# KalistaW/enterprise_warp

Hardware: AMD Instinct MI355X
Metric: lnL evals/sec (whole node), 45-psr CURN batched; % fp64 MFMA peak (higher is better)
Workload: dtype f64; 1 GPU; C3: 45 psr, n=2000..20000 TOAs (495k) over 14.7 yr, ECORR, RN+DM 30 freqs, CURN 14 freqs merged, fixed white noise (TNT cached), basis m=132; global_batch=4096, batch_per_gpu=4096, n_pulsars=45, parallelism=units1

## Files before the change

### enterprise_warp_amd/_lib.py

```python
import ctypes as C
import os

_HERE = os.path.dirname(os.path.abspath(__file__))
CPU_LIB_PATH = os.path.join(_HERE, "libewarp_cpu.so")
BACKEND = os.environ.get("EWARP_BACKEND", "hip").lower()
if BACKEND not in ("hip", "cpu"):
    raise ValueError(f"EWARP_BACKEND={BACKEND!r}: expected 'hip' (default) or 'cpu'")
LIB_PATH = os.environ.get("EWARP_HIP_LIB") or (CPU_LIB_PATH if BACKEND == "cpu" else
                                               os.path.join(_HERE, "libewarp_hip.so"))
DEV_LIB_PATH = os.path.join(_HERE, "libewarp_hip_dev.so")

EWH_ABI_VERSION = 11
COMMON_MAX_TERMS = 16
COMMON_CORRELATED, COMMON_OPTSTAT = 0, 1
SPEC_POWERLAW, SPEC_TURNOVER, SPEC_FREESPEC, SPEC_CONST = 1, 2, 3, 4
DELAY_EXP_DIP, DELAY_YEARLY_SIN = 1, 2


class Pref(C.Structure):
    _fields_ = [("idx", C.c_int32), ("pad_", C.c_int32), ("cval", C.c_double)]


class SpecEntry(C.Structure):
    _fields_ = [("kind", C.c_int32), ("col", C.c_int32), ("p0", Pref), ("p1", Pref), ("p2", Pref),
# ... 29 lines not shown
    _fields_ = [("n_col", C.c_int32), ("orf", _dp), ("spec", C.POINTER(SpecEntry)), ("kind", C.c_int32),
                ("n_term", C.c_int32), ("terms", C.POINTER(CommonTerm))]


class PtaDesc(C.Structure):
    _fields_ = [("abi_version", C.c_int32), ("n_pulsar", C.c_int32), ("n_param", C.c_int32),
                ("white_fixed", C.c_int32), ("pulsars", C.POINTER(PulsarDesc)), ("common", C.POINTER(CommonDesc))]


EXPORTS = ["ewh_create", "ewh_num_devices", "ewh_set_fixed_white", "ewh_lnl_batch", "ewh_lnl_units_device",
           "ewh_keep_dim", "ewh_corr_partial_device", "ewh_corr_finish_device",
           "ewh_last_unit_terms", "ewh_unit_cost", "ewh_set_kernel_mode", "ewh_optstat", "ewh_contract_device",
           "ewh_transfer_stats", "ewh_lat_b_max", "ewh_refine_stats", "ewh_cond_dims", "ewh_cond_gp",
           "ewh_cond_joint_dims", "ewh_cond_joint",
           "ewh_destroy", "ewh_last_error", "ewh_version"]
DEV_EXPORTS = ["ewh_dev_gram", "ewh_dev_reduced", "ewh_dev_images"]

_lib = None


class EngineError(RuntimeError):
    pass


def load():
    global _lib
    if _lib is not None:
        return _lib
    if BACKEND != "cpu":
        try:
            import torch
# ... 52 lines not shown
    lib.ewh_lat_b_max.argtypes = []
    lib.ewh_lat_b_max.restype = C.c_int
    lib.ewh_destroy.argtypes = [C.c_void_p]
    lib.ewh_destroy.restype = None
    lib.ewh_last_error.argtypes = []
    lib.ewh_last_error.restype = C.c_char_p
    lib.ewh_version.argtypes = []
    lib.ewh_version.restype = C.c_int
    if hasattr(lib, "ewh_dev_gram"):
        lib.ewh_dev_gram.argtypes = [C.c_void_p, C.c_int32, _dp, C.c_int32, _dp]
        lib.ewh_dev_gram.restype = C.c_int
        lib.ewh_dev_reduced.argtypes = [C.c_void_p, C.c_int32, _dp, _dp]
        lib.ewh_dev_reduced.restype = C.c_int
        lib.ewh_dev_images.argtypes = [C.c_void_p, C.c_int32, _dp, _dp, _ip]
        lib.ewh_dev_images.restype = C.c_int
    _lib = lib
    return lib


def check(rc):
    if rc != 0:
        raise EngineError(f"libewarp_hip error {rc}: {_lib.ewh_last_error().decode(errors='replace')}")
```

### enterprise_warp_amd/csrc/chol_partial.hip

```cpp
#include "ewarp_dev.h"

namespace ewh_dev {
namespace {

template <int NB, int KEEP>
int launch_partial(const UnitSpan& s, double* keep_out, int keep_bs) {
  if constexpr (partial_in_registers(NB, KEEP) && NB - KEEP >= Split<NB>::H) {
    hipLaunchKernelGGL(HIP_KERNEL_NAME(chol_mfma_kernel<NB, default_waves(NB), PANEL_2L, false, KEEP>),
                       dim3((unsigned)s.n), dim3(64), 0, s.st, s.jobs, s.B, s.u0, s.b_off, s.theta, s.ldth, s.units,
                       keep_out, 0, keep_bs);
    return 0;
  } else {
    return set_err(EWH_E_UNSUPPORTED, "common: reduced basis too narrow for the kept common block");
  }
}

}

int launch_partial_nb(int nb, int keep, const UnitSpan& s, double* keep_out, int keep_bs) {
  if (!partial_in_registers(nb, keep))
    return set_err(EWH_E_UNSUPPORTED, "common: no register kernel for this reduced width and kept size");
#define EWH_PARTK(NBV, KV) \
  case KV: return launch_partial<NBV, KV>(s, keep_out, keep_bs);
#define EWH_PART(NBV)   \
  case NBV:             \
// ... 26 lines not shown
```

### enterprise_warp_amd/csrc/chol_small.hip

```cpp
#include "ewarp_dev.h"

namespace ewh_dev {
namespace {

static_assert(front_map_ok(1) && front_map_ok(2) && front_map_ok(3) && front_map_ok(4) && front_map_ok(5) &&
                  front_map_ok(6) && front_map_ok(7) && front_map_ok(8) && front_map_ok(9),
              "front-pad map: a permutation of the frame, real columns and r in order, pads onto stored pads");
static_assert(MFMA_NB_MAX == 9, "front_map_ok covers every register-kernel width");
static_assert(front_elem_ok(1) && front_elem_ok(2) && front_elem_ok(3) && front_elem_ok(4) && front_elem_ok(5) &&
                  front_elem_ok(6) && front_elem_ok(7) && front_elem_ok(8) && front_elem_ok(9),
              "front_elem: base + constant + lane part == front_src(row) LD + front_src(col)");
static_assert(img_map_ok(1) && img_map_ok(2) && img_map_ok(3), "operand image map, 1..3 blocks");
static_assert(img_map_ok(4) && img_map_ok(5), "operand image map, 4 and 5 blocks");
static_assert(img_map_ok(6), "operand image map, 6 blocks");
static_assert(img_map_ok(7), "operand image map, 7 blocks");
static_assert(img_map_ok(8), "operand image map, 8 blocks");
static_assert(img_map_ok(9), "operand image map, 9 blocks");

template <int NB, int ALG = PANEL_2L, bool STAMP = false, int W = default_waves(NB), bool FULL = false, int DEAD = -1,
          bool IMG = false>
void launch_chol_mfma(const UnitSpan& s) {
  hipLaunchKernelGGL(HIP_KERNEL_NAME(chol_mfma_kernel<NB, W, ALG, STAMP, 0, FULL, DEAD, IMG>), dim3((unsigned)s.n),
                     dim3(64), 0, s.st, s.jobs, s.B, s.u0, s.b_off, s.theta, s.ldth, s.units, nullptr, 0, 0);
}

template <int NB, bool STAMP = false, bool IMG = false>
void launch_chol_front(int dead, const UnitSpan& s) {
  constexpr int W = default_waves(NB);
  switch (front_inst(NB, dead)) {
    case 3: launch_chol_mfma<NB, PANEL_2L, STAMP, W, false, 3, IMG>(s); break;
    case 2: launch_chol_mfma<NB, PANEL_2L, STAMP, W, false, 2, IMG>(s); break;
    case 1: launch_chol_mfma<NB, PANEL_2L, STAMP, W, false, NB == 6 ? -1 : 1, IMG>(s); break;
    default: launch_chol_mfma<NB, PANEL_2L, STAMP, W, false, -1, IMG>(s); break;
  }
}

template <int NB, bool STAMP = false>
void launch_chol_product(int dead, bool img, const UnitSpan& s) {
  if (img)
    launch_chol_front<NB, STAMP, true>(dead, s);
  else
    launch_chol_front<NB, STAMP, false>(dead, s);
}

}

#ifdef EWH_DEV
bool variant_built(int mode) {
  return mode == 15 || mode == 16 || mode == 17 || mode == 19 || mode == 21 || mode == 22 || mode == 23 ||
         mode == 24 || mode == 25 || mode == 26 || mode == 28 || mode == 30 || mode == 31 || mode == 32;
}
extern "C" int ewh_dev_stamps(long long* out, long long n) {
  if (n > (long long)STAMP_UNITS * STAMP_N) n = (long long)STAMP_UNITS * STAMP_N;
  return hipMemcpyFromSymbol(out, HIP_SYMBOL(g_stamps), (size_t)n * sizeof(long long)) == hipSuccess ? 0 : -1;
}
#else
bool variant_built(int) { return false; }
#endif

int launch_chol_small(int mode, int nb, int dead, bool img, const UnitSpan& s) {
#ifdef EWH_DEV
  if (nb == 8) {
    switch (mode) {
      case 17: launch_chol_mfma<8, PANEL_1L>(s); return 0;
      case 21: launch_chol_product<8, true>(dead, img, s); return 0;
      case 26: launch_chol_mfma<8, PANEL_2L, false, 1, true>(s); return 0;
      default: break;
    }
  }
#endif
  switch (nb) {
    case 1: launch_chol_product<1>(dead, img, s); return 0;
    case 2: launch_chol_product<2>(dead, img, s); return 0;
    case 3: launch_chol_product<3>(dead, img, s); return 0;
    case 4: launch_chol_product<4>(dead, img, s); return 0;
    case 5: launch_chol_product<5>(dead, img, s); return 0;
    case 6: launch_chol_product<6>(dead, img, s); return 0;
    case 7: launch_chol_product<7>(dead, img, s); return 0;
    case 8: launch_chol_product<8>(dead, img, s); return 0;
    case 9: launch_chol_product<9>(dead, img, s); return 0;
    default: return set_err(EWH_E_UNSUPPORTED, "no register kernel past 9 blocks");
  }
}

}
```

### enterprise_warp_amd/csrc/ewarp_ctx.h

```cpp
#pragma once

#include "ewarp_launch.h"
#include "ewarp_mem.h"

#include <utility>

namespace ewh_host {

using namespace ewh_dev;
using namespace ewh_mem;

constexpr size_t LDS_MAX = 160 * 1024;

struct PsrHost {
  int n_toa = 0, m = 0, nlead = 0, ld = 0, nb = 0, n_epoch = 0;
  int max_epoch = 0;
  int fx_m = 0, fx_ld = 0, fx_nb = 0;
  int ncommon = 0, nloc = 0, gstart = 0;
  int gstart_v = 0;
  PsrDev dev{};
  int* d_colptr = nullptr;
  DSpec* d_spec = nullptr;
  int* d_fx_colptr = nullptr;
  DSpec* d_fx_spec = nullptr;
  int* d_fx_rep = nullptr;
  int* d_fx_ulist = nullptr;
  int fx_nu = 0;
  URec* d_fx_urec = nullptr;
  std::vector<int> fx_tidx;
  int* d_fx_urep = nullptr;
  double* d_S = nullptr;
  double* d_Slo = nullptr;
  double* d_Srev = nullptr;
  double* d_img = nullptr;
  double* d_imgf = nullptr;
  double* d_Tlo = nullptr;
  bool has_theta_white = false;
  int n_slot = 0;
  ewh_pref* d_slots = nullptr;
  std::vector<ewh_pref> slots;
  DelayDev delay{};
  double *d_Gf = nullptr, *d_Gflo = nullptr, *d_wf = nullptr, *d_betaf = nullptr;
  double fxKb = 0.0;
  int nproj = 0;
  bool has_proj = false;
// ... 163 lines not shown
```

### enterprise_warp_amd/csrc/ewarp_dev.h

```cpp
#pragma once
#include <hip/hip_runtime.h>

#include <algorithm>
#include <cmath>
#include <cstdint>
#include <cstring>
#include <string>
#include <type_traits>
#include <vector>

#include "ewarp_hip.h"
#include "ewarp_route.h"

namespace ewh_dev {

int set_err(int code, const std::string& msg);

#define EWH_HIP(expr)                                                          \
  do {                                                                         \
    hipError_t e_ = (expr);                                                    \
    if (e_ != hipSuccess)                                                      \
      return ::ewh_dev::set_err(EWH_E_HIP, std::string(#expr) + ": " + hipGetErrorString(e_)); \
  } while (0)

#ifdef EWH_DEBUG
#define EWH_DCHECK(cond, what)                                                                           \
  do {                                                                                                   \
// ... 27 lines not shown
}

struct DSpec {
  int kind, col;
  int i0, i1, i2, pad_;
  double v0, v1, v2;
  double a, lnf, lnfyr, f;
};

__device__ __forceinline__ double dpar(int idx, double cval, const double* th) {
  return idx >= 0 ? th[idx] : cval;
}

constexpr double LN10 = 2.302585092994045684;

template <int DUMMY = 0>
__device__ __forceinline__ double spec_phi_body(const DSpec& s, const double* th) {
  switch (s.kind) {
    case EWH_SPEC_POWERLAW: {
      const double lgA = dpar(s.i0, s.v0, th), gam = dpar(s.i1, s.v1, th);
      return exp(s.a + 2.0 * LN10 * lgA + (gam - 3.0) * s.lnfyr - gam * s.lnf);
    }
    case EWH_SPEC_TURNOVER: {
      const double lgA = dpar(s.i0, s.v0, th), gam = dpar(s.i1, s.v1, th);
      double fc = dpar(s.i2, s.v2, th);
      if (fc < 0) fc = exp(LN10 * fc);
      return exp(s.a + 2.0 * LN10 * lgA - 3.0 * s.lnfyr - gam * (log(s.f + fc) - s.lnfyr));
    }
    case EWH_SPEC_FREESPEC:
      return exp(2.0 * LN10 * dpar(s.i0, s.v0, th));
    case EWH_SPEC_CONST:
      return s.v0;
    default:
      return __builtin_nan("");
  }
}
// ... 148 lines not shown
  const DSpec* spec;
  const double* K;
  int kstride;
  int fail;
  const int* rep = nullptr;
  const int* ulist = nullptr;
  int nu = 0;
  const struct URec* urec = nullptr;
  const int* urep = nullptr;
  int ntidx = 0;
  int tidx[16] = {};
  const double* mats_lo = nullptr;
  const double* mats_rev = nullptr;
  const double* img = nullptr;
  const double* img_front = nullptr;
};

struct UnitSpan {
  const CholJob* jobs; int B; long long u0, n; int b_off;
  const double* theta; int ldth; double* units; hipStream_t st;
};

struct URec {
  static constexpr int NE = 3;
  DSpec e[NE];
  int ne, pad_[3];
};
constexpr int STAGE_THETA_MAX = 512;
constexpr int TIDX_MAX = 16;

template <int NB>
__global__ __launch_bounds__(256) void contract_mfma_kernel(PsrDev P, const double* __restrict__ w,
                                                            const double* __restrict__ beta,
                                                            const double* __restrict__ s,
                                                            const double* __restrict__ fac,
                                                            double* __restrict__ G) {
  constexpr int LD = 16 * NB;
  constexpr int NBLK = NB * (NB + 1) / 2;
  constexpr int SLOTS = (NBLK + 3) / 4;
  extern __shared__ __attribute__((aligned(16))) double smem[];
  double* tile = smem;
  double* wt = smem + CT_ROWS * LD;
// ... 388 lines not shown
#pragma unroll
  for (int sk = S0; sk < 4; ++sk) C = __builtin_amdgcn_mfma_f64_16x16x4f64(Ui[sk], Uj[sk], C, 0, 0, 1);
}

constexpr int FRONT_PAD_MAX = 15;
__host__ __device__ constexpr int front_pads(int ld, int mreal) {
  const int s = ld - 1 - mreal;
  return s < 0 ? 0 : s > FRONT_PAD_MAX ? FRONT_PAD_MAX : s;
}
__host__ __device__ constexpr int front_src(int w, int s, int ld) {
  return w < s ? ld - 1 - s + w : w == ld - 1 ? w : w - s;
}
constexpr int front_dead(int ld, int mreal) { return front_pads(ld, mreal) / 4; }
constexpr int front_inst(int nb, int dead) {
  return dead <= 0 || (nb == 6 && dead == 1) ? -1 : dead > 3 ? 3 : dead;
}
constexpr bool front_map_ok(int nb) {
  const int ld = 16 * nb;
  for (int mreal = 0; mreal < ld; ++mreal) {
    const int s = front_pads(ld, mreal);
    int next = 0;
    for (int w = 0; w < ld; ++w) {
      const int a = front_src(w, s, ld);
      if (w < s) {
        if (a != ld - 1 - s + w || a < mreal || a >= ld - 1) return false;
      } else if (w == ld - 1) {
        if (a != ld - 1 || next != ld - 1 - s) return false;
      } else {
        if (a != next++ || a >= ld - 1) return false;
      }
// ... 347 lines not shown
        const double rs = rsqrt_nr(dv);
        hook.on_scale(r, rs);
        static_for<bb + 1, NB>([&](auto JJ) { blk(JJ)[r] *= rs; });
      }
    });
  }
  }
}

#ifdef EWH_DEV
constexpr int STAMP_UNITS = 4096, STAMP_N = 24;
static __device__ long long g_stamps[STAMP_UNITS * STAMP_N];
#endif

template <int NB, int W, int ALG = PANEL_2L, bool STAMP = false, int KEEP = 0, bool FULL = false, int DEAD = -1,
          bool IMG = false>
__global__ __launch_bounds__(64) __attribute__((amdgpu_waves_per_eu(W, W)))
void chol_mfma_kernel(const CholJob* __restrict__ jobs, int B, long long u0, int b_off,
                      const double* __restrict__ theta, int ldth, double* __restrict__ out_units,
                      double* __restrict__ keep_out, int keep_b0, int keep_bs) {
#ifdef EWH_DEV
  long long stp[STAMP_N];
#define EWH_STAMP(I)                                            \
  if constexpr (STAMP) {                                        \
    __builtin_amdgcn_sched_barrier(0);                          \
    stp[(I)] = (long long)__builtin_amdgcn_s_memtime();         \
    __builtin_amdgcn_sched_barrier(0);                          \
  }
#else
  static_assert(!STAMP, "phase stamps exist only in the dev library");
#define EWH_STAMP(I)
#endif
  EWH_STAMP(0)
  constexpr int LD = 16 * NB;
  using S = Split<NB, FULL>;
  constexpr int H = S::H;
  static_assert(!FULL || KEEP == 0, "the FULL form has no kept blocks");
  static_assert(FULL || NB - KEEP >= H, "kept blocks must lie in the phase-3 triangle");
  __shared__ double phinv[LD];
  __shared__ double phs[LD];
  const int lane = threadIdx.x;
  const int q = lane >> 4, c = lane & 15;
  const long long u = u0 + xcd_unit(blockIdx.x, gridDim.x);
  const int p = (int)(u / B), b = (int)(u % B);
  const CholJob J = jobs[p];
  [[maybe_unused]] const gdptr A = (gdptr)(J.mats + (long long)(b - b_off) * J.mstride);
  const double* th = theta + (long long)b * ldth;
  constexpr bool FRONT = DEAD >= 0;
  static_assert(!FRONT || (KEEP == 0 && ALG == PANEL_2L), "front-pad order: the full two-level factorisation");
  static_assert(!IMG || (KEEP == 0 && ALG == PANEL_2L && !FULL), "operand image: the product form without kept blocks");
  typedef double v2d __attribute__((ext_vector_type(2)));
  typedef const __attribute__((address_space(1))) v2d* gv2ptr;
  [[maybe_unused]] const gv2ptr I = IMG ? (gv2ptr)(FRONT ? J.img_front : J.img) + lane : nullptr;
  EWH_DCHECK(!IMG || (I != nullptr && J.mstride == 0), "chol_mfma: the job carries the launch's operand image");
  [[maybe_unused]] auto image_block = [&](auto BI, auto BJ, v4d& v) {
    constexpr long long o = img_index(NB, decltype(BI)::value, decltype(BJ)::value, 0, 0) / 2;
    static_assert(img_index(NB, decltype(BI)::value, decltype(BJ)::value, 2, 0) / 2 == o + 64, "image halves 1 KiB apart");
    const v2d lo = I[o], hi = I[o + 64];
    v[0] = lo.x;
    v[1] = lo.y;
    v[2] = hi.x;
    v[3] = hi.y;
  };
  constexpr bool BLKLD = KEEP == 0 && ALG == PANEL_2L && !FULL;
  const int s = FRONT ? front_pads(LD, __builtin_amdgcn_readfirstlane(J.mreal)) : 0;
  EWH_DCHECK(!FRONT || s >= 4 * DEAD, "chol_mfma: the job has the launch's dead slices");
  [[maybe_unused]] const gdptr Af = front_base<NB>(A, s);

  v4d pre[NB];
  static_for<0, NB>([&](auto BJ) {
    if constexpr (IMG) {
      image_block(std::integral_constant<int, 0>{}, BJ, pre[decltype(BJ)::value]);
    } else {
      static_for<0, 4>([&](auto R) {
        constexpr int r = decltype(R)::value;
        if constexpr (FRONT) {
          pre[decltype(BJ)::value][r] = front_elem<NB, DEAD, 0, decltype(BJ)::value, r>(Af, q, c, s);
        } else {
          pre[decltype(BJ)::value][r] = A[(long long)(q + 4 * r) * LD + 16 * decltype(BJ)::value + c];
        }
      });
    }
  });
  LogAcc ldet;
  if (J.urec != nullptr && (J.ntidx > 0 || ldth <= STAGE_THETA_MAX)) {
    __shared__ double ths[STAGE_THETA_MAX];
    int ur[(LD + 63) / 64];
    static_for<0, (LD + 63) / 64>([&](auto I) {
      constexpr int i = decltype(I)::value;
      const int a = 64 * i + lane - s;
      ur[i] = (a >= 0 && a < J.mreal) ? J.urep[a] : -1;
    });
    if (J.ntidx > 0) {
      if (lane < J.ntidx) ths[lane] = th[jobs[p].tidx[lane]];
    } else {
      for (int i = lane; i < ldth; i += 64) ths[i] = th[i];
    }
    __syncthreads();
    for (int u = lane; u < J.nu; u += 64) {
      const URec& R = J.urec[u];
// ... 285 lines not shown
  int n_term = 0;
  int lds_doubles = 0;
  const double* mat = nullptr;
  const ewh_pref* coef = nullptr;
  const DSpec* spec = nullptr;
  const int* set = nullptr;
};

constexpr int DCB = 64;


int launch_contract_nb(int nb, const PsrDev& P, const double* w, const double* beta, const double* s,
                       const double* fac, double* G, int nb_samples, hipStream_t st, double* Glo = nullptr);
int launch_contract2_nb(int nb, int waves, const PsrDev& P, const double* w, const double* beta, double* s,
                        long long s_stride, double* G, int nb_samples, hipStream_t st, const double* rho = nullptr);
int launch_chol_small(int mode, int nb, int dead, bool img, const UnitSpan& s);
int launch_chol_big_nb(int nb, const UnitSpan& s, double* scr, long long cap);
constexpr int LAT_NB_MAX = 8;
constexpr unsigned long long LAT_STALL_BITS = 0x7ff4dead057a1100ull;
int launch_chol_lat(int nb, int dead, const CholJob* jobs, int B, int P, const double* theta, int ldth, double* units,
                    double* host_units, hipStream_t st, bool stamp = false, int var = 0);
long long wide_scratch_per_wg(int nb, int keep);
long long dd_scratch_per_wg(int ld);
int launch_chol_dd(const UnitSpan& s, double* scr, long long scr_per_wg, long long cap, int ld, bool r05a = false);
int set_dd_attributes();
int launch_verify_units(const double* a, const double* b, long long u0, long long n, int* list, int* count,
                        unsigned long long* total, hipStream_t st, bool all = false);
int launch_count_units(unsigned long long* total, long long n, hipStream_t st);
int launch_chol_dd_list(const UnitSpan& s, double* scr, long long scr_per_wg, long long cap, const int* list,
                        const int* count, int ld, bool r05a = false);
int launch_chol_wide(const UnitSpan& s, double* scr, long long scr_per_wg, long long cap, int keep, double* keep_out,
// ... 9 lines not shown
```

### enterprise_warp_amd/csrc/ewarp_hip.hip

```cpp
#include "ewarp_ctx.h"

#include <atomic>
#include <chrono>
#include <map>
#include <mutex>

namespace ewh_dev {

thread_local std::string g_err;

int set_err(int code, const std::string& msg) {
  g_err = msg;
  return code;
}

__global__ __launch_bounds__(256) void chol_lds_kernel(const CholJob* __restrict__ jobs, int B,
                                                       long long u0, int b_off,
                                                       const double* __restrict__ theta, int ldth,
                                                       double* __restrict__ out_units) {
  extern __shared__ __attribute__((aligned(16))) double sm[];
  __shared__ double red[4];
  const long long u = u0 + blockIdx.x;
  const int p = (int)(u / B), b = (int)(u % B);
  const CholJob J = jobs[p];
// ... 216 lines not shown
    launch_gram_dd_units(ps.dev, ps.nb, (unsigned)std::min<long long>(s.n, 64), ps.d_Tlo, h->var.d_w.p, h->var.d_beta.p,
                         list, count, s.B, s.b_off, h->var.d_G.p, h->var.d_Glo.p, s.st);
    if (ps.delay.n_delay > 0)
      launch_delay_scatter(ps.ld, (int)s.n, h->var.d_dcol.p, h->var.d_dcollo.p, h->var.d_G.p, h->var.d_Glo.p, s.st);
    EWH_HIP(hipGetLastError());
  }
  return launch_chol_dd_list(s, h->d_ddscr.p, per, std::min<long long>(cap, s.n), list, count, 16 * g.nb, false);
}

int partial_units(DevCtx* h, int nb, const UnitSpan& s, double* keep_out) {
  if (partial_route_for(h->plan, nb, h->keep) == PartialRoute::Register)
    return launch_partial_nb(nb, h->keep, s, keep_out, s.B);
  return launch_wide(h, nb, h->keep, s, keep_out);
}

int launch_register(DevCtx* h, const Segment& g) {
  const UnitSpan& s = g.span;
  const int dead = h->osmode ? 0 : front_dead(16 * g.nb, g.mreal);
  bool img = g.src == Source::FixedRun;
  for (long long p = s.u0 / s.B; img && p <= (s.u0 + s.n - 1) / s.B; ++p)
    img = (front_inst(g.nb, dead) >= 1 ? h->psr[p].d_imgf : h->psr[p].d_img) != nullptr;
  return launch_chol_small(h->kernel_mode, g.nb, dead, img, s);
}

int launch_lds(const UnitSpan& s, int mreal) {
  const size_t ma = (size_t)mreal + 1, lds = (ma * (ma + 1) / 2 + ma) * sizeof(double);
  if (lds > LDS_MAX - 64) return set_err(EWH_E_UNSUPPORTED, "reduced matrix too large for the LDS Cholesky kernel");
  hipLaunchKernelGGL(chol_lds_kernel, dim3((unsigned)s.n), dim3(256), lds, s.st, s.jobs, s.B, s.u0, s.b_off, s.theta,
                     s.ldth, s.units);
  return 0;
}

constexpr long long BIG_SLOTS = 2048;

int dispatch_chol(DevCtx* h, const Segment& g) {
  switch (route_for(h->plan, h->corr, h->osmode, g.nb, g.src == Source::FixedRun)) {
    case Route::Register: return launch_register(h, g);
// ... 1204 lines not shown
    (void)hipSetDevice(H->ctx[i]->device);
    (void)hipEventDestroy(H->ev[i]);
  }
  if (H->d_part.p) {
    (void)hipSetDevice(H->ctx[0]->device);
    H->d_part.release();
  }
  for (DevCtx* c : H->ctx) destroy_ctx(c);
  peer_release_all(H);
  H->h_theta.release();
  H->h_out.release();
  delete H;
}

#ifdef EWH_DEV
int ewh_dev_gram(ewh_handle* H, int32_t p, const double* theta_host, int32_t B, double* G_out) {
  DevCtx* h = H->ctx[0];
  if (p < 0 || p >= h->P || B <= 0) return set_err(EWH_E_INVALID, "bad arguments");
  if (h->white_fixed && h->n_delay_psr > 0)
    return set_err(EWH_E_UNSUPPORTED, "ewh_dev_gram: fixed white noise with delay pulsars");
  int rc;
  EWH_HIP(hipSetDevice(h->device));
  const bool wf = h->white_fixed;
  h->white_fixed = false;
  rc = reserve_var_scratch(h, B);
  h->white_fixed = wf;
  if (rc) return rc;
  if (B > h->var.chunk) return set_err(EWH_E_INVALID, "B exceeds the varying-WN chunk");
  if ((rc = reserve_io(h, B))) return rc;
  if (h->n_param > 0)
// ... 62 lines not shown
```

### enterprise_warp_amd/csrc/ewarp_plan.h

```cpp
#pragma once

namespace ewh_dev {

struct KernelPlan {
  bool in_range = true;
  bool valid = true;
  bool variant = false;
  bool lat = true;
  bool lat_stamps = false;
  int lat_variant = 0;
  bool lds_only = false;
  bool all_wide = false;
  bool all_dd = false;
  bool refine = true;
  bool wide_r05a = false;
  bool contract2 = true;
  bool rsep = true;
  int contract2_waves = 0;
  bool epoch_multi = true;
  bool fixed_gram_dd = true;
  bool stage_spectra = true;
  bool minv_reg = true;
  bool corr_right = true;
  bool corr_fuse_diag = true;
  bool corr_fused = true;
  bool corr_pairs = true;
  bool corr_rowupdate_r1 = false;
  bool corr_diag_lds = false;
  bool corr_one_tile = false;
  bool corr_pair_unpiped = false;
  bool corr_trailing = false;
};

constexpr int KERNEL_MODE_MAX = 39;

constexpr KernelPlan plan_for(int mode, bool dev_lib) {
// ... 5 lines not shown
  switch (mode) {
    case 0: p.lat = true; dev_only = false; break;
    case 1:
      p.lds_only = true; p.refine = false;
      p.corr_fused = false; p.corr_rowupdate_r1 = true; p.corr_diag_lds = true;
      dev_only = false;
      break;
    case 2: dev_only = false; break;
    case 7:
      p.contract2 = false; p.fixed_gram_dd = false; p.minv_reg = false;
      p.corr_fused = false; p.corr_diag_lds = true; p.corr_trailing = true;
      dev_only = false;
      break;
    case 27: p.all_wide = true; p.refine = false; dev_only = false; break;
    case 29: p.all_dd = true; dev_only = false; break;
    case 15: p.contract2_waves = 4; p.variant = true; break;
    case 16: p.contract2_waves = 8; p.variant = true; break;
    case 17: case 21: case 26: p.variant = true; break;
    case 19: p.stage_spectra = false; p.variant = true; break;
    case 22: p.lat = true; p.lat_stamps = true; p.variant = true; break;
    case 23: p.lat = true; p.lat_variant = 3; p.variant = true; break;
    case 24: p.lat = true; p.lat_variant = 1; p.variant = true; break;
    case 25: p.lat = true; p.lat_variant = 2; p.variant = true; break;
    case 28: p.corr_pairs = false; p.corr_one_tile = true; p.variant = true; break;
    case 30: p.rsep = false; p.contract2_waves = 30; p.variant = true; break;
    case 31: p.corr_pairs = false; p.variant = true; break;
    case 32: p.corr_pair_unpiped = true; p.variant = true; break;
    case 33: p.corr_fuse_diag = false; break;
    case 34: p.wide_r05a = true; break;
    case 35: p.contract2_waves = 35; break;
    case 36: p.rsep = false; break;
    case 37: p.epoch_multi = false; break;
    case 38: p.rsep = false; p.contract2_waves = 38; break;
    case 39: p.rsep = false; p.contract2_waves = 39; break;
    default: p.valid = false; break;
  }
  if (dev_only && !dev_lib) p.valid = false;
  return p;
}

constexpr bool same_plan(const KernelPlan& a, const KernelPlan& b) {
  return a.in_range == b.in_range && a.valid == b.valid && a.variant == b.variant && a.lat == b.lat &&
         a.lat_stamps == b.lat_stamps && a.lat_variant == b.lat_variant && a.lds_only == b.lds_only && a.all_wide == b.all_wide &&
         a.all_dd == b.all_dd && a.refine == b.refine && a.wide_r05a == b.wide_r05a && a.contract2 == b.contract2 &&
         a.rsep == b.rsep && a.contract2_waves == b.contract2_waves && a.epoch_multi == b.epoch_multi &&
         a.fixed_gram_dd == b.fixed_gram_dd && a.stage_spectra == b.stage_spectra && a.minv_reg == b.minv_reg &&
         a.corr_right == b.corr_right && a.corr_fuse_diag == b.corr_fuse_diag && a.corr_fused == b.corr_fused &&
         a.corr_pairs == b.corr_pairs && a.corr_rowupdate_r1 == b.corr_rowupdate_r1 &&
         a.corr_diag_lds == b.corr_diag_lds && a.corr_one_tile == b.corr_one_tile &&
         a.corr_pair_unpiped == b.corr_pair_unpiped && a.corr_trailing == b.corr_trailing;
}

constexpr KernelPlan batched_default_plan() {
  KernelPlan p;
  p.lat = false;
  p.corr_right = false;
  return p;
}

static_assert(same_plan(plan_for(0, false), KernelPlan{}) && same_plan(plan_for(0, true), KernelPlan{}),
              "mode 0 is the default plan");
static_assert(same_plan(plan_for(2, false), batched_default_plan()),
              "mode 2 leaves the latency path and (with every non-default mode) the right-looking schedule, no more");
static_assert(!plan_for(-1, true).in_range && !plan_for(KERNEL_MODE_MAX + 1, true).in_range &&
                  plan_for(3, true).in_range && plan_for(KERNEL_MODE_MAX, false).in_range,
              "the range of mode numbers");
static_assert(!plan_for(-1, true).valid && !plan_for(3, true).valid && !plan_for(18, true).valid &&
                  !plan_for(20, true).valid && !plan_for(KERNEL_MODE_MAX + 1, true).valid,
              "a mode outside the lists is invalid");
static_assert(plan_for(33, true).valid && !plan_for(33, false).valid && !plan_for(15, false).valid &&
                  !plan_for(39, false).valid,
              "a dev-only mode is invalid in the product library");
static_assert(plan_for(1, false).valid && plan_for(7, false).valid && plan_for(27, false).valid &&
                  plan_for(29, false).valid,
              "the product modes");

}
```

### enterprise_warp_amd/csrc/ewarp_setup.hip

```cpp
#include "ewarp_ctx.h"
#include "ewarp_desc.h"

#include <map>

using namespace ewh_host;

namespace {

int nb_for(int cols_with_r) { return (cols_with_r + 15) / 16; }

bool pref_uses_theta(const ewh_pref& r) { return r.idx >= 0; }

DSpec to_dspec(const ewh_spec_entry& e, int col) {
  DSpec d{};
  d.kind = e.kind;
  d.col = col;
  d.i0 = e.p0.idx; d.i1 = e.p1.idx; d.i2 = e.p2.idx;
  d.v0 = e.p0.cval; d.v1 = e.p1.cval; d.v2 = e.p2.cval;
  d.f = e.f;
  d.lnf = e.f > 0 ? std::log(e.f) : 0.0;
  d.lnfyr = e.fyr > 0 ? std::log(e.fyr) : 0.0;
  d.a = e.df > 0 ? std::log(e.df / (12.0 * M_PI * M_PI)) : 0.0;
  return d;
}
// ... 301 lines not shown
    jobs[p].mats_lo = ps.d_Slo;
    if (ps.d_Slo) {
      launch_rev_input(ps.d_S, ps.d_Slo, ps.d_Srev, (long long)ps.fx_ld * ps.fx_ld, h->stream);
      EWH_HIP(hipGetLastError());
      jobs[p].mats_rev = ps.d_Srev;
    }
    if (ps.d_img) {
      launch_operand_image(ps.d_S, ps.fx_nb, front_pads(ps.fx_ld, mreal), ps.d_img, ps.d_imgf, h->stream);
      EWH_HIP(hipGetLastError());
      jobs[p].img = ps.d_img;
      jobs[p].img_front = ps.d_imgf;
    }
    if (jobs[p].urec != nullptr) {
      jobs[p].ntidx = (int)ps.fx_tidx.size();
      for (int i = 0; i < jobs[p].ntidx; ++i) jobs[p].tidx[i] = ps.fx_tidx[i];
    }
  }
  EWH_HIP(hipMemcpyAsync(fails.data(), h->d_fxfail, sizeof(int) * h->P, hipMemcpyDeviceToHost, h->stream));
  EWH_HIP(hipStreamSynchronize(h->stream));
  for (int p = 0; p < h->P; ++p) jobs[p].fail = fails[p];
  EWH_HIP(hipMemcpy(h->d_jobs_fixed, jobs.data(), sizeof(CholJob) * h->P, hipMemcpyHostToDevice));
  return 0;
}

void destroy_ctx(DevCtx* h) {
  if (!h) return;
  (void)hipSetDevice(h->device);
  if (h->stream) (void)hipStreamSynchronize(h->stream);
  drop_graphs(h);
  h->h_stage.release();
// ... 215 lines not shown
    std::vector<DSpec> ent;
    if (corr_var) build_csr_mapped(s, vpos, ps.m, pad0, pad1, ptr, ent);
    else build_csr(s, 0, s.n_col, ptr, ent);
    if ((rc = dupload(h, &ps.d_colptr, ptr.data(), ptr.size()))) return bail(rc);
    if ((rc = dupload(h, &ps.d_spec, ent.data(), ent.size()))) return bail(rc);
    build_csr_fixed(s, ps.nlead, ps.nloc, ps.gstart, ps.fx_ld, ptr, ent);
    if ((rc = dupload(h, &ps.d_fx_colptr, ptr.data(), ptr.size()))) return bail(rc);
    if ((rc = dupload(h, &ps.d_fx_spec, ent.data(), ent.size()))) return bail(rc);
    {
      std::vector<int> rep, ulist;
      build_spec_rep(ptr, ent, rep, ulist);
      ps.fx_nu = (int)ulist.size();
      std::vector<int> urep(rep.size(), -1), uidx(rep.size(), -1);
      for (size_t u = 0; u < ulist.size(); ++u) uidx[ulist[u]] = (int)u;
      bool fits = true;
      std::vector<URec> urec(std::max<size_t>(1, ulist.size()));
      for (size_t u = 0; u < ulist.size(); ++u) {
        const int a = ulist[u];
        const int ne = ptr[a + 1] - ptr[a];
        if (ne > URec::NE) fits = false;
        urec[u] = URec{};
        urec[u].ne = std::min(ne, URec::NE);
        for (int e = 0; e < urec[u].ne; ++e) urec[u].e[e] = ent[ptr[a] + e];
      }
      std::vector<int> tl;
      for (size_t u = 0; u < ulist.size(); ++u)
        for (int e = 0; e < urec[u].ne; ++e)
          for (int idx : {urec[u].e[e].i0, urec[u].e[e].i1, urec[u].e[e].i2})
            if (idx >= 0 && std::find(tl.begin(), tl.end(), idx) == tl.end()) tl.push_back(idx);
      std::sort(tl.begin(), tl.end());
// ... 1 lines not shown
      if (fits && (int)tl.size() <= TIDX_MAX) {
        ps.fx_tidx = tl;
        auto pos = [&](int idx) { return idx < 0 ? idx : (int)(std::lower_bound(tl.begin(), tl.end(), idx) - tl.begin()); };
        for (size_t u = 0; u < ulist.size(); ++u)
          for (int e = 0; e < urec[u].ne; ++e) {
            urec[u].e[e].i0 = pos(urec[u].e[e].i0);
            urec[u].e[e].i1 = pos(urec[u].e[e].i1);
            urec[u].e[e].i2 = pos(urec[u].e[e].i2);
          }
      }
      for (size_t a = 0; a < rep.size(); ++a)
        if (ptr[a] < ptr[a + 1]) urep[a] = uidx[rep[a]];
      if (fits) {
        if ((rc = dupload(h, &ps.d_fx_urec, urec.data(), urec.size()))) return bail(rc);
        if ((rc = dupload(h, &ps.d_fx_urep, urep.data(), urep.size()))) return bail(rc);
      }
      if (ulist.empty()) ulist.push_back(0);
      if ((rc = dupload(h, &ps.d_fx_rep, rep.data(), rep.size()))) return bail(rc);
      if ((rc = dupload(h, &ps.d_fx_ulist, ulist.data(), ulist.size()))) return bail(rc);
    }
  }
  h->white_fixed = (d->white_fixed != 0) && !any_theta_white;
  if ((rc = dalloc(h, &h->d_jobs_fixed, h->P))) return bail(rc);
  if ((rc = dalloc(h, &h->d_jobs_var, h->P))) return bail(rc);
  h->osmode = d->common && d->common->kind == EWH_COMMON_OPTSTAT;
  if (h->osmode && !h->white_fixed)
    return bail(set_err(EWH_E_UNSUPPORTED, "optimal statistic: white noise must be fixed (TNT cached)"));
  if (h->white_fixed && (rc = setup_fixed(h))) return bail(rc);
  if (d->common && (rc = setup_common(h, d))) return bail(rc);
  if (h->white_fixed && !h->corr && !h->osmode) {
// ... 15 lines not shown
```

Baseline: 1.201 million lnL evals/s.

## Add compact powerlaw-record prologue to small Cholesky kernel for fixed-white runs

Packs each pulsar's fixed spectrum entries into compact 160-byte powerlaw-only records. The small MFMA Cholesky kernel loads them straight into registers and evaluates phi per unique column in parallel across lanes, instead of staging theta and generic DSpec records through shared memory. It also replaces the 64-bit unit divide/modulo with a 32-bit magic-number decode. The aim is a cheaper per-unit prologue, paid for with more kernel instantiations, register pressure from the cached records, and a powerlaw-only restriction that falls back to the old path otherwise.

After: 1.221 million lnL evals/s (median of 6 runs). 1.02x the previous value.

```diff
diff --git a/enterprise_warp_amd/_lib.py b/enterprise_warp_amd/_lib.py
--- a/enterprise_warp_amd/_lib.py
+++ b/enterprise_warp_amd/_lib.py
@@ -67,7 +67,7 @@
            "ewh_transfer_stats", "ewh_lat_b_max", "ewh_refine_stats", "ewh_cond_dims", "ewh_cond_gp",
            "ewh_cond_joint_dims", "ewh_cond_joint",
            "ewh_destroy", "ewh_last_error", "ewh_version"]
-DEV_EXPORTS = ["ewh_dev_gram", "ewh_dev_reduced", "ewh_dev_images"]
+DEV_EXPORTS = ["ewh_dev_gram", "ewh_dev_reduced", "ewh_dev_images", "ewh_dev_prologue_launches"]
 
 _lib = None
 
@@ -150,6 +150,9 @@
         lib.ewh_dev_reduced.restype = C.c_int
         lib.ewh_dev_images.argtypes = [C.c_void_p, C.c_int32, _dp, _dp, _ip]
         lib.ewh_dev_images.restype = C.c_int
+    if hasattr(lib, "ewh_dev_prologue_launches"):
+        lib.ewh_dev_prologue_launches.argtypes = [C.POINTER(C.c_int64)]
+        lib.ewh_dev_prologue_launches.restype = C.c_int
     _lib = lib
     return lib
 
diff --git a/enterprise_warp_amd/csrc/chol_partial.hip b/enterprise_warp_amd/csrc/chol_partial.hip
--- a/enterprise_warp_amd/csrc/chol_partial.hip
+++ b/enterprise_warp_amd/csrc/chol_partial.hip
@@ -8,7 +8,7 @@
   if constexpr (partial_in_registers(NB, KEEP) && NB - KEEP >= Split<NB>::H) {
     hipLaunchKernelGGL(HIP_KERNEL_NAME(chol_mfma_kernel<NB, default_waves(NB), PANEL_2L, false, KEEP>),
                        dim3((unsigned)s.n), dim3(64), 0, s.st, s.jobs, s.B, s.u0, s.b_off, s.theta, s.ldth, s.units,
-                       keep_out, 0, keep_bs);
+                       keep_out, 0, keep_bs, UnitDec{});
     return 0;
   } else {
     return set_err(EWH_E_UNSUPPORTED, "common: reduced basis too narrow for the kept common block");
diff --git a/enterprise_warp_amd/csrc/chol_small.hip b/enterprise_warp_amd/csrc/chol_small.hip
--- a/enterprise_warp_amd/csrc/chol_small.hip
+++ b/enterprise_warp_amd/csrc/chol_small.hip
@@ -1,4 +1,4 @@
-#include "ewarp_dev.h"
+#include "ewarp_chol_small.h"
 
 namespace ewh_dev {
 namespace {
@@ -17,30 +17,12 @@
 static_assert(img_map_ok(8), "operand image map, 8 blocks");
 static_assert(img_map_ok(9), "operand image map, 9 blocks");
 
-template <int NB, int ALG = PANEL_2L, bool STAMP = false, int W = default_waves(NB), bool FULL = false, int DEAD = -1,
-          bool IMG = false>
-void launch_chol_mfma(const UnitSpan& s) {
-  hipLaunchKernelGGL(HIP_KERNEL_NAME(chol_mfma_kernel<NB, W, ALG, STAMP, 0, FULL, DEAD, IMG>), dim3((unsigned)s.n),
-                     dim3(64), 0, s.st, s.jobs, s.B, s.u0, s.b_off, s.theta, s.ldth, s.units, nullptr, 0, 0);
-}
-
-template <int NB, bool STAMP = false, bool IMG = false>
-void launch_chol_front(int dead, const UnitSpan& s) {
-  constexpr int W = default_waves(NB);
-  switch (front_inst(NB, dead)) {
-    case 3: launch_chol_mfma<NB, PANEL_2L, STAMP, W, false, 3, IMG>(s); break;
-    case 2: launch_chol_mfma<NB, PANEL_2L, STAMP, W, false, 2, IMG>(s); break;
-    case 1: launch_chol_mfma<NB, PANEL_2L, STAMP, W, false, NB == 6 ? -1 : 1, IMG>(s); break;
-    default: launch_chol_mfma<NB, PANEL_2L, STAMP, W, false, -1, IMG>(s); break;
-  }
-}
-
 template <int NB, bool STAMP = false>
-void launch_chol_product(int dead, bool img, const UnitSpan& s) {
-  if (img)
-    launch_chol_front<NB, STAMP, true>(dead, s);
+void launch_chol_product(int dead, bool img, bool pl, const UnitSpan& s) {
+  if (pl)
+    launch_chol_small_pl(NB, dead, img, STAMP, s);
   else
-    launch_chol_front<NB, STAMP, false>(dead, s);
+    launch_chol_images<NB, STAMP, false>(dead, img, s);
 }
 
 }
@@ -48,37 +30,43 @@
 #ifdef EWH_DEV
 bool variant_built(int mode) {
   return mode == 15 || mode == 16 || mode == 17 || mode == 19 || mode == 21 || mode == 22 || mode == 23 ||
-         mode == 24 || mode == 25 || mode == 26 || mode == 28 || mode == 30 || mode == 31 || mode == 32;
+         mode == 24 || mode == 25 || mode == 26 || mode == 28 || mode == 30 || mode == 31 || mode == 32 || mode == 14;
 }
+int dev_stamps_pl(long long* out, long long n);
+static bool g_stamps_in_pl = false;
 extern "C" int ewh_dev_stamps(long long* out, long long n) {
   if (n > (long long)STAMP_UNITS * STAMP_N) n = (long long)STAMP_UNITS * STAMP_N;
+  if (g_stamps_in_pl) return dev_stamps_pl(out, n);
   return hipMemcpyFromSymbol(out, HIP_SYMBOL(g_stamps), (size_t)n * sizeof(long long)) == hipSuccess ? 0 : -1;
 }
 #else
 bool variant_built(int) { return false; }
 #endif
 
-int launch_chol_small(int mode, int nb, int dead, bool img, const UnitSpan& s) {
+int launch_chol_small(int mode, int nb, int dead, bool img, bool pl, const UnitSpan& s) {
 #ifdef EWH_DEV
   if (nb == 8) {
     switch (mode) {
       case 17: launch_chol_mfma<8, PANEL_1L>(s); return 0;
-      case 21: launch_chol_product<8, true>(dead, img, s); return 0;
+      case 21:
+        g_stamps_in_pl = pl;
+        launch_chol_product<8, true>(dead, img, pl, s);
+        return 0;
       case 26: launch_chol_mfma<8, PANEL_2L, false, 1, true>(s); return 0;
       default: break;
     }
   }
 #endif
   switch (nb) {
-    case 1: launch_chol_product<1>(dead, img, s); return 0;
-    case 2: launch_chol_product<2>(dead, img, s); return 0;
-    case 3: launch_chol_product<3>(dead, img, s); return 0;
-    case 4: launch_chol_product<4>(dead, img, s); return 0;
-    case 5: launch_chol_product<5>(dead, img, s); return 0;
-    case 6: launch_chol_product<6>(dead, img, s); return 0;
-    case 7: launch_chol_product<7>(dead, img, s); return 0;
-    case 8: launch_chol_product<8>(dead, img, s); return 0;
-    case 9: launch_chol_product<9>(dead, img, s); return 0;
+    case 1: launch_chol_product<1>(dead, img, pl, s); return 0;
+    case 2: launch_chol_product<2>(dead, img, pl, s); return 0;
+    case 3: launch_chol_product<3>(dead, img, pl, s); return 0;
+    case 4: launch_chol_product<4>(dead, img, pl, s); return 0;
+    case 5: launch_chol_product<5>(dead, img, pl, s); return 0;
+    case 6: launch_chol_product<6>(dead, img, pl, s); return 0;
+    case 7: launch_chol_product<7>(dead, img, pl, s); return 0;
+    case 8: launch_chol_product<8>(dead, img, pl, s); return 0;
+    case 9: launch_chol_product<9>(dead, img, pl, s); return 0;
     default: return set_err(EWH_E_UNSUPPORTED, "no register kernel past 9 blocks");
   }
 }
diff --git a/enterprise_warp_amd/csrc/chol_small_pl.hip b/enterprise_warp_amd/csrc/chol_small_pl.hip
--- /dev/null
+++ b/enterprise_warp_amd/csrc/chol_small_pl.hip
@@ -0,0 +1,29 @@
+#include "ewarp_chol_small.h"
+
+namespace ewh_dev {
+
+#ifdef EWH_DEV
+int dev_stamps_pl(long long* out, long long n) {
+  return hipMemcpyFromSymbol(out, HIP_SYMBOL(g_stamps), (size_t)n * sizeof(long long)) == hipSuccess ? 0 : -1;
+}
+#endif
+
+void launch_chol_small_pl(int nb, int dead, bool img, [[maybe_unused]] bool stamp, const UnitSpan& s) {
+#ifdef EWH_DEV
+  if (stamp && nb == 8) return launch_chol_images<8, true, true>(dead, img, s);
+#endif
+  switch (nb) {
+    case 1: return launch_chol_images<1, false, true>(dead, img, s);
+    case 2: return launch_chol_images<2, false, true>(dead, img, s);
+    case 3: return launch_chol_images<3, false, true>(dead, img, s);
+    case 4: return launch_chol_images<4, false, true>(dead, img, s);
+    case 5: return launch_chol_images<5, false, true>(dead, img, s);
+    case 6: return launch_chol_images<6, false, true>(dead, img, s);
+    case 7: return launch_chol_images<7, false, true>(dead, img, s);
+    case 8: return launch_chol_images<8, false, true>(dead, img, s);
+    case 9: return launch_chol_images<9, false, true>(dead, img, s);
+    default: return;
+  }
+}
+
+}
diff --git a/enterprise_warp_amd/csrc/ewarp_chol_small.h b/enterprise_warp_amd/csrc/ewarp_chol_small.h
--- /dev/null
+++ b/enterprise_warp_amd/csrc/ewarp_chol_small.h
@@ -0,0 +1,36 @@
+#pragma once
+#include "ewarp_dev.h"
+
+namespace ewh_dev {
+namespace {
+
+template <int NB, int ALG = PANEL_2L, bool STAMP = false, int W = default_waves(NB), bool FULL = false, int DEAD = -1,
+          bool IMG = false, bool PL = false>
+void launch_chol_mfma(const UnitSpan& s) {
+  constexpr bool PLB = PL && pl_built(NB, DEAD, IMG);
+  hipLaunchKernelGGL(HIP_KERNEL_NAME(chol_mfma_kernel<NB, W, ALG, STAMP, 0, FULL, DEAD, IMG, PLB>), dim3((unsigned)s.n),
+                     dim3(64), 0, s.st, s.jobs, s.B, s.u0, s.b_off, s.theta, s.ldth, s.units, nullptr, 0, 0,
+                     PLB ? unit_dec_make(s.u0, s.B) : UnitDec{});
+}
+
+template <int NB, bool STAMP = false, bool IMG = false, bool PL = false>
+void launch_chol_front(int dead, const UnitSpan& s) {
+  constexpr int W = default_waves(NB);
+  switch (front_inst(NB, dead)) {
+    case 3: launch_chol_mfma<NB, PANEL_2L, STAMP, W, false, 3, IMG, PL>(s); break;
+    case 2: launch_chol_mfma<NB, PANEL_2L, STAMP, W, false, 2, IMG, PL>(s); break;
+    case 1: launch_chol_mfma<NB, PANEL_2L, STAMP, W, false, NB == 6 ? -1 : 1, IMG, PL>(s); break;
+    default: launch_chol_mfma<NB, PANEL_2L, STAMP, W, false, -1, IMG, PL>(s); break;
+  }
+}
+
+template <int NB, bool STAMP = false, bool PL = false>
+void launch_chol_images(int dead, bool img, const UnitSpan& s) {
+  if (img)
+    launch_chol_front<NB, STAMP, true, PL>(dead, s);
+  else
+    launch_chol_front<NB, STAMP, false, PL>(dead, s);
+}
+
+}
+}
diff --git a/enterprise_warp_amd/csrc/ewarp_ctx.h b/enterprise_warp_amd/csrc/ewarp_ctx.h
--- a/enterprise_warp_amd/csrc/ewarp_ctx.h
+++ b/enterprise_warp_amd/csrc/ewarp_ctx.h
@@ -29,6 +29,8 @@
   URec* d_fx_urec = nullptr;
   std::vector<int> fx_tidx;
   int* d_fx_urep = nullptr;
+  PlRec* d_fx_pl = nullptr;
+  int fx_pl_ne = 0;
   double* d_S = nullptr;
   double* d_Slo = nullptr;
   double* d_Srev = nullptr;
diff --git a/enterprise_warp_amd/csrc/ewarp_dev.h b/enterprise_warp_amd/csrc/ewarp_dev.h
--- a/enterprise_warp_amd/csrc/ewarp_dev.h
+++ b/enterprise_warp_amd/csrc/ewarp_dev.h
@@ -11,6 +11,7 @@
 
 #include "ewarp_hip.h"
 #include "ewarp_route.h"
+#include "ewarp_spec.h"
 
 namespace ewh_dev {
 
@@ -68,12 +69,16 @@
 
 constexpr double LN10 = 2.302585092994045684;
 
+__device__ __forceinline__ double powerlaw_phi(double a, double lgA, double gam, double lnfyr, double lnf) {
+  return exp(a + 2.0 * LN10 * lgA + (gam - 3.0) * lnfyr - gam * lnf);
+}
+
 template <int DUMMY = 0>
 __device__ __forceinline__ double spec_phi_body(const DSpec& s, const double* th) {
   switch (s.kind) {
     case EWH_SPEC_POWERLAW: {
       const double lgA = dpar(s.i0, s.v0, th), gam = dpar(s.i1, s.v1, th);
-      return exp(s.a + 2.0 * LN10 * lgA + (gam - 3.0) * s.lnfyr - gam * s.lnf);
+      return powerlaw_phi(s.a, lgA, gam, s.lnfyr, s.lnf);
     }
     case EWH_SPEC_TURNOVER: {
       const double lgA = dpar(s.i0, s.v0, th), gam = dpar(s.i1, s.v1, th);
@@ -252,6 +257,8 @@
   const double* mats_rev = nullptr;
   const double* img = nullptr;
   const double* img_front = nullptr;
+  const PlRec* pl = nullptr;
+  int pl_ne = 0;
 };
 
 struct UnitSpan {
@@ -264,6 +271,7 @@
   DSpec e[NE];
   int ne, pad_[3];
 };
+static_assert(PL_NE == URec::NE, "a compact record (ewarp_spec.h) holds what a staged record holds");
 constexpr int STAGE_THETA_MAX = 512;
 constexpr int TIDX_MAX = 16;
 
@@ -682,6 +690,9 @@
 constexpr int front_dead(int ld, int mreal) { return front_pads(ld, mreal) / 4; }
 constexpr int front_inst(int nb, int dead) {
   return dead <= 0 || (nb == 6 && dead == 1) ? -1 : dead > 3 ? 3 : dead;
+}
+constexpr bool pl_built(int nb, int inst, bool img) {
+  return !(img && ((nb == 6 && inst == 2) || (nb == 8 && inst == -1)));
 }
 constexpr bool front_map_ok(int nb) {
   const int ld = 16 * nb;
@@ -1059,11 +1070,11 @@
 #endif
 
 template <int NB, int W, int ALG = PANEL_2L, bool STAMP = false, int KEEP = 0, bool FULL = false, int DEAD = -1,
-          bool IMG = false>
+          bool IMG = false, bool PL = false>
 __global__ __launch_bounds__(64) __attribute__((amdgpu_waves_per_eu(W, W)))
 void chol_mfma_kernel(const CholJob* __restrict__ jobs, int B, long long u0, int b_off,
                       const double* __restrict__ theta, int ldth, double* __restrict__ out_units,
-                      double* __restrict__ keep_out, int keep_b0, int keep_bs) {
+                      double* __restrict__ keep_out, int keep_b0, int keep_bs, UnitDec ud) {
 #ifdef EWH_DEV
   long long stp[STAMP_N];
 #define EWH_STAMP(I)                                            \
@@ -1086,8 +1097,15 @@
   __shared__ double phs[LD];
   const int lane = threadIdx.x;
   const int q = lane >> 4, c = lane & 15;
-  const long long u = u0 + xcd_unit(blockIdx.x, gridDim.x);
-  const int p = (int)(u / B), b = (int)(u % B);
+  static_assert(!PL || (KEEP == 0 && ALG == PANEL_2L && !FULL), "fixed-form prologue: the product form without kept blocks");
+  int p, b;
+  if constexpr (PL) {
+    unit_decode(ud, (uint32_t)xcd_unit(blockIdx.x, gridDim.x), (uint32_t)B, p, b);
+  } else {
+    const long long u = u0 + xcd_unit(blockIdx.x, gridDim.x);
+    p = (int)(u / B);
+    b = (int)(u % B);
+  }
   const CholJob J = jobs[p];
   [[maybe_unused]] const gdptr A = (gdptr)(J.mats + (long long)(b - b_off) * J.mstride);
   const double* th = theta + (long long)b * ldth;
@@ -1112,6 +1130,28 @@
   EWH_DCHECK(!FRONT || s >= 4 * DEAD, "chol_mfma: the job has the launch's dead slices");
   [[maybe_unused]] const gdptr Af = front_base<NB>(A, s);
 
+  constexpr int CT = (LD + 63) / 64;
+  constexpr int RT = (LD - 1 + 63) / 64;
+  [[maybe_unused]] v2d rc[RT][PL_PIECES - 1] = {};
+  [[maybe_unused]] int urp[CT];
+  [[maybe_unused]] const int pl_nu = PL ? __builtin_amdgcn_readfirstlane(J.nu) : 0;
+  [[maybe_unused]] const int pl_ne = PL ? __builtin_amdgcn_readfirstlane(J.pl_ne) : 0;
+  if constexpr (PL) {
+    EWH_DCHECK(J.pl != nullptr && J.urep != nullptr && pl_ne <= PL_NE && pl_nu <= 64 * RT,
+               "chol_mfma: the job carries the launch's compact records");
+    const gv2ptr R = (gv2ptr)J.pl + lane * PL_PIECES;
+    static_for<0, RT>([&](auto T) {
+      constexpr int t = decltype(T)::value;
+      if (t == 0 || 64 * t < pl_nu)
+        static_for<0, PL_PIECES - 1>([&](auto K) { rc[t][decltype(K)::value] = R[64 * t * PL_PIECES + decltype(K)::value]; });
+    });
+    static_for<0, CT>([&](auto I) {
+      constexpr int i = decltype(I)::value;
+      const int a = 64 * i + lane - s;
+      urp[i] = (a >= 0 && a < J.mreal) ? J.urep[a] : -1;
+    });
+  }
+
   v4d pre[NB];
   static_for<0, NB>([&](auto BJ) {
     if constexpr (IMG) {
@@ -1128,7 +1168,45 @@
     }
   });
   LogAcc ldet;
-  if (J.urec != nullptr && (J.ntidx > 0 || ldth <= STAGE_THETA_MAX)) {
+  if constexpr (PL) {
+    __shared__ double phq[64 * RT];
+    const gdptr thg = (gdptr)th;
+    static_for<0, RT>([&](auto T) {
+      constexpr int t = decltype(T)::value;
+      if (t == 0 || 64 * t < pl_nu) {
+        double lgA[PL_NE], gam[PL_NE];
+        static_for<0, PL_NE>([&](auto E) {
+          constexpr int e = decltype(E)::value;
+          const v2d h = rc[t][pl_piece(e, 0)];
+          const int i0 = __double2loint(h.x), i1 = __double2hiint(h.x);
+          const double t0 = thg[max(i0, 0)], t1 = thg[max(i1, 0)];
+          lgA[e] = i0 >= 0 ? t0 : h.y;
+          gam[e] = i1 >= 0 ? t1 : rc[t][pl_piece(e, 1)].x;
+        });
+        double ph = 0.0;
+        static_for<0, PL_NE>([&](auto E) {
+          constexpr int e = decltype(E)::value;
+          if (e == 0 || e < pl_ne)
+            ph += powerlaw_phi(rc[t][pl_piece(e, 1)].y, lgA[e], gam[e], rc[t][pl_piece(e, 2)].y, rc[t][pl_piece(e, 2)].x);
+        });
+        phq[64 * t + lane] = ph;
+      }
+    });
+    __syncthreads();
+    static_for<0, CT>([&](auto I) {
+      constexpr int i = decltype(I)::value;
+      const int a = 64 * i + lane;
+      if (a < LD) {
+        double pi = 0.0;
+        if (urp[i] >= 0) {
+          const double ph = phq[urp[i]];
+          pi = 1.0 / ph;
+          ldet.add(ph);
+        }
+        phinv[a] = pi;
+      }
+    });
+  } else if (J.urec != nullptr && (J.ntidx > 0 || ldth <= STAGE_THETA_MAX)) {
     __shared__ double ths[STAGE_THETA_MAX];
     int ur[(LD + 63) / 64];
     static_for<0, (LD + 63) / 64>([&](auto I) {
@@ -1444,7 +1522,8 @@
                        const double* fac, double* G, int nb_samples, hipStream_t st, double* Glo = nullptr);
 int launch_contract2_nb(int nb, int waves, const PsrDev& P, const double* w, const double* beta, double* s,
                         long long s_stride, double* G, int nb_samples, hipStream_t st, const double* rho = nullptr);
-int launch_chol_small(int mode, int nb, int dead, bool img, const UnitSpan& s);
+int launch_chol_small(int mode, int nb, int dead, bool img, bool pl, const UnitSpan& s);
+void launch_chol_small_pl(int nb, int dead, bool img, bool stamp, const UnitSpan& s);
 int launch_chol_big_nb(int nb, const UnitSpan& s, double* scr, long long cap);
 constexpr int LAT_NB_MAX = 8;
 constexpr unsigned long long LAT_STALL_BITS = 0x7ff4dead057a1100ull;
diff --git a/enterprise_warp_amd/csrc/ewarp_hip.hip b/enterprise_warp_amd/csrc/ewarp_hip.hip
--- a/enterprise_warp_amd/csrc/ewarp_hip.hip
+++ b/enterprise_warp_amd/csrc/ewarp_hip.hip
@@ -254,13 +254,23 @@
   return launch_wide(h, nb, h->keep, s, keep_out);
 }
 
+#ifdef EWH_DEV
+std::atomic<long long> g_prologue_launches[2] = {{0}, {0}};
+#endif
+
 int launch_register(DevCtx* h, const Segment& g) {
   const UnitSpan& s = g.span;
   const int dead = h->osmode ? 0 : front_dead(16 * g.nb, g.mreal);
   bool img = g.src == Source::FixedRun;
   for (long long p = s.u0 / s.B; img && p <= (s.u0 + s.n - 1) / s.B; ++p)
     img = (front_inst(g.nb, dead) >= 1 ? h->psr[p].d_imgf : h->psr[p].d_img) != nullptr;
-  return launch_chol_small(h->kernel_mode, g.nb, dead, img, s);
+  bool pl = g.src == Source::FixedRun && h->plan.compact_spectra && h->stage_spectra;
+  for (long long p = s.u0 / s.B; pl && p <= (s.u0 + s.n - 1) / s.B; ++p) pl = h->psr[p].d_fx_pl != nullptr;
+  pl = pl && pl_built(g.nb, front_inst(g.nb, dead), img);
+#ifdef EWH_DEV
+  g_prologue_launches[pl ? 1 : 0]++;
+#endif
+  return launch_chol_small(h->kernel_mode, g.nb, dead, img, pl, s);
 }
 
 int launch_lds(const UnitSpan& s, int mreal) {
@@ -1495,6 +1505,11 @@
 }
 
 #ifdef EWH_DEV
+int ewh_dev_prologue_launches(long long* out) {
+  out[0] = g_prologue_launches[0].load();
+  out[1] = g_prologue_launches[1].load();
+  return 0;
+}
 int ewh_dev_gram(ewh_handle* H, int32_t p, const double* theta_host, int32_t B, double* G_out) {
   DevCtx* h = H->ctx[0];
   if (p < 0 || p >= h->P || B <= 0) return set_err(EWH_E_INVALID, "bad arguments");
diff --git a/enterprise_warp_amd/csrc/ewarp_plan.h b/enterprise_warp_amd/csrc/ewarp_plan.h
--- a/enterprise_warp_amd/csrc/ewarp_plan.h
+++ b/enterprise_warp_amd/csrc/ewarp_plan.h
@@ -20,6 +20,7 @@
   bool epoch_multi = true;
   bool fixed_gram_dd = true;
   bool stage_spectra = true;
+  bool compact_spectra = true;
   bool minv_reg = true;
   bool corr_right = true;
   bool corr_fuse_diag = true;
@@ -55,6 +56,7 @@
       break;
     case 27: p.all_wide = true; p.refine = false; dev_only = false; break;
     case 29: p.all_dd = true; dev_only = false; break;
+    case 14: p.compact_spectra = false; p.variant = true; break;
     case 15: p.contract2_waves = 4; p.variant = true; break;
     case 16: p.contract2_waves = 8; p.variant = true; break;
     case 17: case 21: case 26: p.variant = true; break;
@@ -85,7 +87,8 @@
          a.lat_stamps == b.lat_stamps && a.lat_variant == b.lat_variant && a.lds_only == b.lds_only && a.all_wide == b.all_wide &&
          a.all_dd == b.all_dd && a.refine == b.refine && a.wide_r05a == b.wide_r05a && a.contract2 == b.contract2 &&
          a.rsep == b.rsep && a.contract2_waves == b.contract2_waves && a.epoch_multi == b.epoch_multi &&
-         a.fixed_gram_dd == b.fixed_gram_dd && a.stage_spectra == b.stage_spectra && a.minv_reg == b.minv_reg &&
+         a.fixed_gram_dd == b.fixed_gram_dd && a.stage_spectra == b.stage_spectra && a.compact_spectra == b.compact_spectra &&
+         a.minv_reg == b.minv_reg &&
          a.corr_right == b.corr_right && a.corr_fuse_diag == b.corr_fuse_diag && a.corr_fused == b.corr_fused &&
          a.corr_pairs == b.corr_pairs && a.corr_rowupdate_r1 == b.corr_rowupdate_r1 &&
          a.corr_diag_lds == b.corr_diag_lds && a.corr_one_tile == b.corr_one_tile &&
@@ -106,6 +109,9 @@
 static_assert(!plan_for(-1, true).in_range && !plan_for(KERNEL_MODE_MAX + 1, true).in_range &&
                   plan_for(3, true).in_range && plan_for(KERNEL_MODE_MAX, false).in_range,
               "the range of mode numbers");
+static_assert(plan_for(14, true).valid && !plan_for(14, true).compact_spectra && plan_for(14, true).stage_spectra &&
+                  plan_for(19, true).compact_spectra && !plan_for(14, false).valid,
+              "mode 14 turns off the fixed-form prologue alone, in the dev library");
 static_assert(!plan_for(-1, true).valid && !plan_for(3, true).valid && !plan_for(18, true).valid &&
                   !plan_for(20, true).valid && !plan_for(KERNEL_MODE_MAX + 1, true).valid,
               "a mode outside the lists is invalid");
diff --git a/enterprise_warp_amd/csrc/ewarp_setup.hip b/enterprise_warp_amd/csrc/ewarp_setup.hip
--- a/enterprise_warp_amd/csrc/ewarp_setup.hip
+++ b/enterprise_warp_amd/csrc/ewarp_setup.hip
@@ -339,6 +339,8 @@
     if (jobs[p].urec != nullptr) {
       jobs[p].ntidx = (int)ps.fx_tidx.size();
       for (int i = 0; i < jobs[p].ntidx; ++i) jobs[p].tidx[i] = ps.fx_tidx[i];
+      jobs[p].pl = ps.d_fx_pl;
+      jobs[p].pl_ne = ps.fx_pl_ne;
     }
   }
   EWH_HIP(hipMemcpyAsync(fails.data(), h->d_fxfail, sizeof(int) * h->P, hipMemcpyDeviceToHost, h->stream));
@@ -584,6 +586,8 @@
       std::vector<int> urep(rep.size(), -1), uidx(rep.size(), -1);
       for (size_t u = 0; u < ulist.size(); ++u) uidx[ulist[u]] = (int)u;
       bool fits = true;
+      std::vector<PlRec> plrec;
+      const bool compact = pl_pack(ptr, ent, ulist, h->n_param, plrec, &ps.fx_pl_ne);
       std::vector<URec> urec(std::max<size_t>(1, ulist.size()));
       for (size_t u = 0; u < ulist.size(); ++u) {
         const int a = ulist[u];
@@ -615,6 +619,7 @@
       if (fits) {
         if ((rc = dupload(h, &ps.d_fx_urec, urec.data(), urec.size()))) return bail(rc);
         if ((rc = dupload(h, &ps.d_fx_urep, urep.data(), urep.size()))) return bail(rc);
+        if (compact && (rc = dupload(h, &ps.d_fx_pl, plrec.data(), plrec.size()))) return bail(rc);
       }
       if (ulist.empty()) ulist.push_back(0);
       if ((rc = dupload(h, &ps.d_fx_rep, rep.data(), rep.size()))) return bail(rc);
diff --git a/enterprise_warp_amd/csrc/ewarp_spec.h b/enterprise_warp_amd/csrc/ewarp_spec.h
--- /dev/null
+++ b/enterprise_warp_amd/csrc/ewarp_spec.h
@@ -0,0 +1,106 @@
+#pragma once
+#include <cstddef>
+#include <cstdint>
+#include <limits>
+#include <vector>
+
+#if defined(__HIPCC__)
+#define EWH_SPEC_HD __host__ __device__
+#else
+#define EWH_SPEC_HD
+#endif
+
+namespace ewh_dev {
+
+constexpr int PL_KIND_POWERLAW = 1;
+constexpr int PL_NE = 3;
+constexpr int PL_LANES = 64;
+
+struct PlEntry {
+  int32_t i0, i1;
+  double v0;
+  double v1, a;
+  double lnf, lnfyr;
+};
+
+struct PlRec {
+  PlEntry e[PL_NE];
+  int32_t ne, pad_[3];
+};
+
+static_assert(sizeof(PlEntry) == 48 && sizeof(PlRec) == 160 && alignof(PlRec) == 8, "compact record: 10 x 16 bytes");
+static_assert(offsetof(PlEntry, i0) == 0 && offsetof(PlEntry, i1) == 4 && offsetof(PlEntry, v0) == 8 &&
+                  offsetof(PlEntry, v1) == 16 && offsetof(PlEntry, a) == 24 && offsetof(PlEntry, lnf) == 32 &&
+                  offsetof(PlEntry, lnfyr) == 40,
+              "entry: {i0, i1, v0} {v1, a} {lnf, lnfyr}");
+static_assert(offsetof(PlRec, e) == 0 && offsetof(PlRec, ne) == 144, "record: three entries, then ne");
+constexpr int PL_PIECES = 10;
+constexpr int pl_piece(int e, int k) { return 3 * e + k; }
+static_assert(pl_piece(PL_NE - 1, 2) == PL_PIECES - 2 && PL_PIECES * 16 == (int)sizeof(PlRec), "pieces cover the record");
+
+inline PlEntry pl_pad_entry() {
+  return PlEntry{-1, -1, 0.0, 0.0, -std::numeric_limits<double>::infinity(), 0.0, 0.0};
+}
+inline PlRec pl_pad_rec() {
+  PlRec r{};
+  for (int e = 0; e < PL_NE; ++e) r.e[e] = pl_pad_entry();
+  r.ne = 0;
+  return r;
+}
+
+constexpr size_t pl_padded(size_t nu) { return nu == 0 ? PL_LANES : (nu + PL_LANES - 1) / PL_LANES * PL_LANES; }
+
+template <class Spec>
+bool pl_pack(const std::vector<int>& ptr, const std::vector<Spec>& ent, const std::vector<int>& ulist, int n_param,
+             std::vector<PlRec>& out, int* ne_max) {
+  out.clear();
+  *ne_max = 0;
+  if (n_param < 1) return false;
+  auto fail = [&] {
+    out.clear();
+    *ne_max = 0;
+    return false;
+  };
+  out.assign(pl_padded(ulist.size()), pl_pad_rec());
+  for (size_t u = 0; u < ulist.size(); ++u) {
+    const int a = ulist[u];
+    const int ne = ptr[a + 1] - ptr[a];
+    if (ne > PL_NE) return fail();
+    for (int e = 0; e < ne; ++e) {
+      const Spec& s = ent[ptr[a] + e];
+      if (s.kind != PL_KIND_POWERLAW || s.i0 >= n_param || s.i1 >= n_param) return fail();
+      out[u].e[e] = PlEntry{s.i0 < 0 ? -1 : s.i0, s.i1 < 0 ? -1 : s.i1, s.v0, s.v1, s.a, s.lnf, s.lnfyr};
+    }
+    out[u].ne = ne;
+    if (ne > *ne_max) *ne_max = ne;
+  }
+  return true;
+}
+
+struct UnitDec {
+  int32_t p0 = 0;
+  uint32_t r0 = 0, magic = 0;
+};
+
+inline UnitDec unit_dec_make(long long u0, int B) {
+  UnitDec d;
+  d.p0 = (int32_t)(u0 / B);
+  d.r0 = (uint32_t)(u0 % B);
+  const uint64_t m = (uint64_t(1) << 32) / (uint32_t)B;
+  d.magic = m > 0xffffffffull ? 0xffffffffu : (uint32_t)m;
+  return d;
+}
+
+EWH_SPEC_HD inline void unit_decode(const UnitDec& d, uint32_t v, uint32_t B, int& p, int& b) {
+  const uint32_t t = d.r0 + v;
+  uint32_t q = (uint32_t)(((uint64_t)t * d.magic) >> 32);
+  uint32_t r = t - q * B;
+  if (r >= B) {
+    q += 1;
+    r -= B;
+  }
+  p = d.p0 + (int)q;
+  b = (int)r;
+}
+
+}
```
